# jlk9/MPAS-Ocean.jl

Hardware: AMD Instinct MI355X
Metric: cell-updates/sec per RK4 step (higher is better)
Workload: dtype f64

## Files before the change

include/moka_hip.h:

```cpp
#ifndef MOKA_HIP_H
#define MOKA_HIP_H
#include <stdint.h>

#ifdef __cplusplus
extern "C" {
#endif

typedef struct moka_ctx   moka_ctx;
typedef struct moka_plan  moka_plan;
typedef struct moka_mesh  moka_mesh;
typedef struct moka_state moka_state;

typedef enum {
    MOKA_OK = 0,
    MOKA_ERR_ARG = -1,
    MOKA_ERR_HIP = -2,
    MOKA_ERR_NO_DEVICE = -3,
    MOKA_ERR_ALLOC = -4,
    MOKA_ERR_UNSUPPORTED = -5,
    MOKA_ERR_COMM = -6
} moka_status;

typedef enum {
    MOKA_ORDER_DEFAULT = 0,
// ... 95 lines not shown
int  moka_mesh_info_get(const moka_mesh *mesh, moka_mesh_info *info);

int moka_gradient_on_edge(moka_mesh *mesh, const double *scalarCell, double *gradEdge);
int moka_divergence_on_cell(moka_mesh *mesh, const double *vecEdge, double *tempEdge, double *divCell);
int moka_curl_on_vertex(moka_mesh *mesh, const double *vecEdge, double *curlVertex);
int moka_interpolate_cell2edge(moka_mesh *mesh, const double *cellValue, double *edgeValue, int nlev);

int moka_gradient_on_edge_vjp(moka_mesh *mesh, double *dGradEdge , double *dScalarCell );
int moka_gradient_on_edge_jvp(moka_mesh *mesh, const double *dScalarCell, double *dGradEdge);
int moka_divergence_on_cell_vjp(moka_mesh *mesh, double *dDivCell , double *dVecEdge ,
                                double *dTempEdge );
int moka_divergence_on_cell_jvp(moka_mesh *mesh, const double *dVecEdge, double *dTempEdge , double *dDivCell);
int moka_curl_on_vertex_vjp(moka_mesh *mesh, const double *dCurlVertex, double *dVecEdge );
int moka_curl_on_vertex_jvp(moka_mesh *mesh, const double *dVecEdge, double *dCurlVertex );

int  moka_state_create(moka_ctx *ctx, moka_mesh *mesh, moka_state **out);
void moka_state_destroy(moka_state *st);
int  moka_state_upload(moka_state *st, int field, int time_level, const double *host);
int  moka_state_download(moka_state *st, int field, int time_level, double *host);

int  moka_state_download_rows(moka_state *st, int field, int time_level, int64_t nRows, const int32_t *rows, double *host);

int  moka_state_array_address(moka_state *st, int field, int time_level, uint64_t *address);

int  moka_state_optimize_placement(moka_state *st, int max_tries, double *ms_before, double *ms_after);
typedef struct { int32_t field; double ms_old, ms_new; int32_t kept; } moka_placement_trial;
int  moka_state_placement_log(const moka_state *st, int32_t capacity, moka_placement_trial *out, int32_t *n);
int64_t moka_state_placement_launches(const moka_state *st);

int moka_advance_time_levels(moka_state *st, int flags);
int moka_diagnostic_compute(moka_state *st, int flags);
int moka_compute_normal_velocity_tendency(moka_state *st, int flags);
int moka_compute_layer_thickness_tendency(moka_state *st, int flags);
int moka_tendencies(moka_state *st);
int moka_step_fe(moka_state *st, double dt, int flags);
int moka_step_rk4(moka_state *st, double dt);
int moka_run(moka_state *st, int integrator, double dt, int64_t nsteps, int flags);
int moka_sum_sq(moka_state *st, int field, int time_level, double *out);

typedef struct moka_halo moka_halo;
int  moka_ctx_streams(moka_ctx *ctx, void **compute_stream, void **comm_stream);
int  moka_mesh_permutation(const moka_mesh *mesh, int kind, int32_t *new_to_old);
int  moka_mesh_class_ranges(const moka_mesh *mesh, int32_t capacity, int32_t *nClasses, int32_t *patchStart,
                            int32_t *cellStart, int32_t *edgeStart);
int  moka_halo_create(moka_state *st, int32_t nNeighbors, const int32_t *sendCells, const int64_t *sendCellOff,
                      const int32_t *sendEdges, const int64_t *sendEdgeOff, const int32_t *recvCells,
// ... 158 lines not shown
```

mpas-ocean.jl_amd/csrc/api.hip:

```cpp
#include <hip/hip_runtime.h>

#include <algorithm>
#include <atomic>
#include <climits>
#include <cmath>
#include <cstdio>
#include <cstdlib>
#include <cstring>
#include <map>
#include <new>
#include <string>
#include <utility>
#include <vector>

#include "state.hpp"

namespace moka {

void fill_mesh_info(const Plan &p, moka_mesh_info *info);

struct TuningEntry {
    int mask, max;
    std::atomic<int> value;
    TuningEntry(int def, int m, int x) : mask(m), max(x), value(def) {}
    bool accepts(int v) const { return mask ? (v & ~mask) == 0 : v >= 0 && v <= max; }
};
static TuningEntry g_tuning[] = {
    {0, 0, -1},
    {1 << 0, 0x7f | 1 << 10 | 1 << 11, 0},
    {1, 0, 1},
    {1, 0, 1},
    {1, 0, 1},
    {0, 0, 3},
    {0, 0, INT_MAX},
    {0, 0, 1},
    {1 << 0 | 1 << 1 | 1 << 7, 0xf | 7 << 7 | 1 << 16, 0},
    {1, 0, 1},
};
constexpr int N_TUNING = sizeof(g_tuning) / sizeof(g_tuning[0]);

int tuning(TuningKey key) { return g_tuning[key].value.load(); }

}

namespace mk {

int fail(moka_ctx *ctx, int code, const std::string &msg)
{
    set_error(msg);
    if (ctx) ctx->err = msg;
    return code;
}

int lanes_per_column(int K)
{
    int l = 1;
    while (l < K && l < 64) l <<= 1;
    return l;
}

// ... 288 lines not shown
    const uint32_t rowB = 480;
    const int64_t nRows = bytes / rowB, nFetch = nRows / 4;
    uint32_t *sink = reinterpret_cast<uint32_t *>(static_cast<unsigned char *>(buf) + bytes);
    double best = 0.0;
    hipError_t rc = hipMemsetAsync(buf, 0x5A, (size_t)bytes + 64, s);
    for (int i = 0; i < iters && rc == hipSuccess; ++i) {
        if ((rc = hipEventRecord(ctx->ev0, s)) != hipSuccess) break;
        if ((rc = launch_bw_gather_n(buf, nRows, rowB, nFetch, sink, ctx->nCUs, s)) != hipSuccess) break;
        if ((rc = hipEventRecord(ctx->ev1, s)) != hipSuccess) break;
        if ((rc = hipEventSynchronize(ctx->ev1)) != hipSuccess) break;
        float ms = 0.f;
        if ((rc = hipEventElapsedTime(&ms, ctx->ev0, ctx->ev1)) != hipSuccess) break;
        best = std::max(best, (double)nFetch * rowB / ((double)ms * 1e-3) / 1e9);
    }
    (void)hipStreamSynchronize(s);
    (void)hipFree(buf);
    HIPCHK(ctx, rc);
    *gbs = best;
    return MOKA_OK;
}

int moka_set_tuning(int key, int value)
{
    if (key < 1 || key >= N_TUNING) return fail(nullptr, MOKA_ERR_ARG, "unknown tuning key");
    if (!g_tuning[key].accepts(value)) return fail(nullptr, MOKA_ERR_ARG, "tuning key " + std::to_string(key) + ": value names no kernel instance");
    g_tuning[key].value.store(value);
    return MOKA_OK;
}

int moka_get_tuning(int key, int *value)
{
    if (!value) return fail(nullptr, MOKA_ERR_ARG, "value is NULL");
    if (key < 1 || key >= N_TUNING) return fail(nullptr, MOKA_ERR_ARG, "unknown tuning key");
    *value = g_tuning[key].value.load();
    return MOKA_OK;
}

int moka_kernel_variant_available(int variant)
{
    return variant == 0 || variant == 3 || variant == 4 || variant == 11;
}

int moka_set_kernel_variant(moka_ctx *ctx, int variant)
{
    if (!ctx) return fail(nullptr, MOKA_ERR_ARG, "ctx is NULL");
    if (variant < 0 || variant > 14) return fail(ctx, MOKA_ERR_ARG, "variant must be 0..14");
    if (!moka_kernel_variant_available(variant))
        return fail(ctx, MOKA_ERR_UNSUPPORTED, "this kernel variant was an experiment of rounds 1-3 and no longer exists (0, 3, 4, 11 do)");
    ctx->variant = variant;
    return MOKA_OK;
}

int moka_mesh_create(moka_ctx *ctx, const moka_mesh_desc *desc, moka_mesh **out)
{
    if (!ctx || !out) return fail(ctx, MOKA_ERR_ARG, "NULL argument");
    *out = nullptr;
// ... 252 lines not shown
```

mpas-ocean.jl_amd/csrc/api_state.hip:

```cpp
#include <hip/hip_runtime.h>

#include <algorithm>
#include <cmath>
#include <climits>
#include <cstdint>
#include <mutex>
#include <new>
#include <string>
#include <unordered_set>
#include <utility>
#include <vector>

#include "state.hpp"
#include "tapes.hpp"

namespace mk {

static std::mutex g_liveMutex;
static std::unordered_set<const moka_state *> g_liveStates;
void state_attach(moka_state *st, bool halo)
{
    std::lock_guard<std::mutex> lk(g_liveMutex);
    if (g_liveStates.count(st)) { ++st->attached; st->halos += halo; }
}
bool state_detach(moka_state *st, bool halo)
{
    std::lock_guard<std::mutex> lk(g_liveMutex);
    const bool alive = g_liveStates.count(st) != 0;
    if (alive) { --st->attached; st->halos -= halo; }
    return alive;
}

int ensure_rk_bufs(moka_state *st)
{
    if (st->rk[1].ssh) return MOKA_OK;
    const Plan &p = st->mesh->plan;
    LevelBufs tmp[2];
    const size_t mark = st->mem.mark();
    const size_t sb = st->f32 ? 4 : 8;
    int rc = MOKA_OK;
    for (auto &r : tmp) {
        if (rc == MOKA_OK) rc = st->mem.alloc(&r.u, (size_t)p.K * p.nE, sb);
        if (rc == MOKA_OK) rc = st->mem.alloc(&r.h, (size_t)p.K * p.nC, sb);
        if (rc == MOKA_OK) rc = st->mem.alloc(&r.ssh, (size_t)p.nC, sb);
    }
    if (rc != MOKA_OK) {
        st->mem.rollback(mark);
        return rc;
    }
    st->rk[0] = tmp[0]; st->rk[1] = tmp[1];
    st->phys[2] = tmp[0]; st->phys[3] = tmp[1];
    return MOKA_OK;
}

int ensure_spare(moka_state *st)
{
    if (st->spare.ssh) return MOKA_OK;
    const Plan &p = st->mesh->plan;
    LevelBufs tmp;
    const size_t mark = st->mem.mark();
    const size_t sb = st->f32 ? 4 : 8;
    int rc = st->mem.alloc(&tmp.u, (size_t)p.K * p.nE, sb);
    if (rc == MOKA_OK) rc = st->mem.alloc(&tmp.h, (size_t)p.K * p.nC, sb);
    if (rc == MOKA_OK) rc = st->mem.alloc(&tmp.ssh, (size_t)p.nC, sb);
    if (rc != MOKA_OK) {
        st->mem.rollback(mark);
        return rc;
    }
    st->spare = tmp;
    st->phys[4] = tmp;
    return MOKA_OK;
}

LevelBufs &fe_new_level(moka_state *st) { return st->spare.ssh ? st->spare : st->lev[0]; }

void fe_rotate_levels(moka_state *st)
{
    if (st->spare.ssh) {
        const LevelBufs oldPrev = st->lev[0];
        st->lev[0] = st->lev[1];
// ... 427 lines not shown
int moka_state_create(moka_ctx *ctx, moka_mesh *mesh, moka_state **out)
{
    if (!ctx || !mesh || !out) return fail(ctx, MOKA_ERR_ARG, "NULL argument");
    *out = nullptr;
    moka_state *st = new (std::nothrow) moka_state();
    if (!st) return fail(ctx, MOKA_ERR_ALLOC, "out of host memory");
    st->ctx = ctx;
    st->mem.ctx = ctx;
    st->mesh = mesh;
    const Plan &p = mesh->plan;
    HIPCHK(ctx, hipSetDevice(ctx->device));
    const size_t nEK = (size_t)p.K * p.nE, nCK = (size_t)p.K * p.nC, nVK = (size_t)p.K * p.nV;
    st->f32 = p.stateBytes == 4;
    const MeshDev launchDev = launch_bounds(mesh);
    if (st->f32 && !stage_f32_supported(launchDev)) {
        delete st;
        return fail(ctx, MOKA_ERR_UNSUPPORTED,
                    "fp32-storage state: needs nVertLevels % 4 == 0, nVertLevels <= 128, fields below 4 GiB and patches whose "
                    "records + own u rows fit 64 KB of LDS (smaller patch_cells)");
    }
    const size_t sb = st->f32 ? 4 : 8;
    int rc = MOKA_OK;
    auto A = [&](double **q, size_t n, size_t eb = 8) { if (rc == MOKA_OK) rc = st->mem.alloc(q, n, eb); };
    for (auto &l : st->lev) { A(&l.ssh, p.nC, sb); A(&l.u, nEK, sb); A(&l.h, nCK, sb); }
    A(&st->hEdge[0], nEK, sb); A(&st->hEdge[1], nEK, sb);
    A(&st->F, nEK, sb); A(&st->div, nCK, sb); A(&st->vort, nVK, sb);
    A(&st->tendU, nEK, sb); A(&st->tendH, nCK, sb);
    A(&st->scalar, 2);
    if (rc != MOKA_OK) { moka_state_destroy(st); return rc; }
    st->phys[0] = st->lev[0]; st->phys[1] = st->lev[1];
    HIPCHK(ctx, hipStreamSynchronize(ctx->stream));
    {
        std::lock_guard<std::mutex> lk(g_liveMutex);
        g_liveStates.insert(st);
    }
    *out = st;
    return MOKA_OK;
}

void moka_state_destroy(moka_state *st)
{
    if (!st) return;
    {
        std::lock_guard<std::mutex> lk(g_liveMutex);
        g_liveStates.erase(st);
    }
    (void)hipSetDevice(st->ctx->device);
// ... 511 lines not shown
```

mpas-ocean.jl_amd/csrc/halo.hip:

```cpp
#include <fcntl.h>
#include <sys/mman.h>
#include <sys/stat.h>
#include <unistd.h>

#include <algorithm>
#include <chrono>
#include <cerrno>
#include <cstring>
#include <new>
#include <string>
#include <thread>
#include <vector>

#include "state.hpp"

using namespace mk;

namespace {

struct PushDst {
    unsigned char *u, *h, *ssh;
};

struct PeerLink {
// ... 242 lines not shown
                     const int64_t *recvCellOff, const int32_t *recvEdges, const int64_t *recvEdgeOff,
                     int32_t nPatchesBoundary, int32_t nPatchesOwned, moka_halo **out)
{
    if (!st || !out || nNeighbors < 0 || !sendCellOff || !sendEdgeOff || !recvCellOff || !recvEdgeOff)
        return fail(st ? st->ctx : nullptr, MOKA_ERR_ARG, "NULL argument");
    *out = nullptr;
    const Plan &p = st->mesh->plan;
    if (st->viscDel4 != 0.0)
        return fail(st->ctx, MOKA_ERR_UNSUPPORTED, "Del4 mixing: not on a state with a halo (its stencil reaches three cell rings, the nonlinear halo two)");
    if (st->nTracers > 0) return fail(st->ctx, MOKA_ERR_UNSUPPORTED, "tracers: whole meshes only (no halo; moka_set_tracers(st, 0) first)");
    if (mom_vmix_on(st)) return fail(st->ctx, MOKA_ERR_UNSUPPORTED, "vertical momentum mixing: whole meshes only (no halo; switch the pass off first)");
    if (st->forcedTapes > 0) return fail(st->ctx, MOKA_ERR_UNSUPPORTED, "a moka_forced_tape of this state exists: whole meshes only (no halo)");
    if (nNeighbors > 60) return fail(st->ctx, MOKA_ERR_ARG, "at most 60 neighbours");
    if (nPatchesBoundary < 0 || nPatchesOwned < nPatchesBoundary || nPatchesOwned > p.nPatches)
        return fail(st->ctx, MOKA_ERR_ARG, "patch ranges must satisfy 0 <= boundary <= owned <= nPatches");
    {
        const auto &cp = p.classPatchStart;
        const bool okB = std::find(cp.begin(), cp.end(), nPatchesBoundary) != cp.end();
        const bool okO = std::find(cp.begin(), cp.end(), nPatchesOwned) != cp.end();
        if (!okB || !okO)
            return fail(st->ctx, MOKA_ERR_ARG, "boundary / owned patch counts must be class boundaries of the mesh (moka_mesh_class_ranges)");
    }
    HIPCHK(st->ctx, hipSetDevice(st->ctx->device));
    if (int rc = ensure_rk_bufs(st)) return rc;
    if (int rc = ensure_spare(st)) return rc;
    moka_halo *h = new (std::nothrow) moka_halo();
    if (!h) return fail(st->ctx, MOKA_ERR_ALLOC, "out of host memory");
    h->st = st;
    h->mem.ctx = st->ctx;
    h->nNbr = nNeighbors;
    h->pBoundary = nPatchesBoundary; h->pOwned = nPatchesOwned;
    h->pFirst = nPatchesBoundary;
    h->overlapB = nPatchesBoundary > 0 && nPatchesOwned - nPatchesBoundary < 12000;
    int rc = MOKA_OK;
    try {
        if ((rc = build_halo_map(h, nNeighbors, sendCells, sendCellOff, sendEdges, sendEdgeOff, &h->sendMap, &h->nSend)) ||
            (rc = build_halo_map(h, nNeighbors, recvCells, recvCellOff, recvEdges, recvEdgeOff, &h->recvMap, &h->nRecv))) {
            moka_halo_destroy(h);
            return rc;
        }
        h->peers.resize(nNeighbors);
        h->recvCellStart.assign(nNeighbors, 0); h->recvCellCount.assign(nNeighbors, 0);
        h->recvEdgeStart.assign(nNeighbors, 0); h->recvEdgeCount.assign(nNeighbors, 0);
        h->sendCellCount.resize(nNeighbors); h->sendEdgeCount.resize(nNeighbors);
        for (int i = 0; i < nNeighbors; ++i) {
            h->sendCellCount[i] = (int32_t)(sendCellOff[i + 1] - sendCellOff[i]);
// ... 167 lines not shown
}

int moka_halo_set_acquire(moka_halo *h, int on)
{
    if (!h) return fail(nullptr, MOKA_ERR_ARG, "halo is NULL");
    h->acquireFence = on != 0;
    return MOKA_OK;
}

int moka_halo_direct_available(const moka_halo *h)
{
    return h && h->directOk ? 1 : 0;
}

int moka_halo_export(moka_halo *h, int32_t nbr, int32_t shared, moka_halo_peer_info *out)
{
    if (!h || !out) return fail(h ? h->st->ctx : nullptr, MOKA_ERR_ARG, "NULL argument");
    if (nbr < 0 || nbr >= h->nNbr) return hfail(h, MOKA_ERR_ARG, "neighbour index out of range");
    if (!h->directOk) return hfail(h, MOKA_ERR_UNSUPPORTED, "direct halo transport unavailable: " + h->directWhy);
    moka_state *st = h->st;
    HIPCHK(st->ctx, hipSetDevice(st->ctx->device));
    if (int rc = ensure_flags(h, shared != 0)) return rc;
    if (shared && h->shmName.empty()) return hfail(h, MOKA_ERR_ARG, "the flag block of this halo was created process-local");
    std::memset(out, 0, sizeof *out);
    for (int t = 0; t < moka_state::NPHYS; ++t) {
        void *ptrs[3] = {st->phys[t].u, st->phys[t].h, st->phys[t].ssh};
        for (int f = 0; f < 3; ++f) {
            out->ptr[3 * t + f] = (uint64_t)(uintptr_t)ptrs[f];
            if (shared) {
                hipIpcMemHandle_t hd;
                HIPCHK(st->ctx, hipIpcGetMemHandle(&hd, ptrs[f]));
                static_assert(sizeof hd <= sizeof out->ipc[0], "IPC handle larger than its slot");
                std::memcpy(out->ipc[3 * t + f], &hd, sizeof hd);
            }
        }
    }
    out->flagPtr = (uint64_t)(uintptr_t)h->flags;
    std::strncpy(out->shmName, h->shmName.c_str(), sizeof out->shmName - 1);
    out->dstCell = h->recvCellStart[nbr]; out->dstEdge = h->recvEdgeStart[nbr];
    out->nCells = h->recvCellCount[nbr]; out->nEdges = h->recvEdgeCount[nbr];
    out->slot = nbr;
    out->nNeighbors = h->nNbr;
    out->pid = (int32_t)getpid();
    out->device = st->ctx->device;
    out->stateBytes = st->f32 ? 4 : 8;
    out->nVertLevels = st->mesh->plan.K;
// ... 478 lines not shown
```

mpas-ocean.jl_amd/csrc/inspect.hip:

```cpp
#include <algorithm>

#include "state.hpp"

using namespace mk;

namespace {

template <class T>
__global__ __launch_bounds__(256) void k_gather_rows(double *dst, const T *src, const int32_t *rows, int64_t n, int K)
{
    const int64_t total = n * K;
    for (int64_t i = (int64_t)blockIdx.x * 256 + threadIdx.x; i < total; i += (int64_t)gridDim.x * 256) {
        const int64_t r = i / K;
        const int k = (int)(i - r * K);
        dst[i] = (double)src[(int64_t)rows[r] * K + k];
    }
}

}

extern "C" int moka_state_download_rows(moka_state *st, int field, int time_level, int64_t nRows, const int32_t *rows, double *host)
{
    if (!st || (nRows > 0 && (!rows || !host)) || nRows < 0) return fail(st ? st->ctx : nullptr, MOKA_ERR_ARG, "NULL argument or nRows < 0");
    moka_ctx *c = st->ctx;
// ... 54 lines not shown
    hipError_t e = hipMemcpyAsync(dRows, lib.data(), (size_t)nRows * sizeof(int32_t), hipMemcpyHostToDevice, s);
    if (e == hipSuccess) {
        const unsigned blocks = (unsigned)std::min<int64_t>((nRows * K + 255) / 256, 16384);
        if (st->f32) hipLaunchKernelGGL(k_gather_rows<float>, dim3(blocks), dim3(256), 0, s, dOut, reinterpret_cast<const float *>(src), dRows, nRows, K);
        else hipLaunchKernelGGL(k_gather_rows<double>, dim3(blocks), dim3(256), 0, s, dOut, src, dRows, nRows, K);
        e = hipGetLastError();
    }
    if (e == hipSuccess) e = hipMemcpyAsync(host, dOut, (size_t)nRows * K * sizeof(double), hipMemcpyDeviceToHost, s);
    if (e == hipSuccess) e = hipStreamSynchronize(s);
    if (e != hipSuccess) return done(fail(c, MOKA_ERR_HIP, std::string("moka_state_download_rows: ") + hipGetErrorString(e)));
    return done(MOKA_OK);
}

extern "C" int moka_state_array_address(moka_state *st, int field, int time_level, uint64_t *address)
{
    if (!st || !address) return fail(st ? st->ctx : nullptr, MOKA_ERR_ARG, "NULL argument");
    if (time_level < 0 || time_level > 3 || field < MOKA_F_SSH || field > MOKA_F_LAYER_THICKNESS)
        return fail(st->ctx, MOKA_ERR_ARG, "prognostic fields, time_level 0..3");
    const LevelBufs &b = time_level < 2 ? st->lev[time_level] : st->rk[time_level - 2];
    const double *q = field == MOKA_F_SSH ? b.ssh : field == MOKA_F_NORMAL_VELOCITY ? b.u : b.h;
    *address = (uint64_t)(uintptr_t)q;
    return MOKA_OK;
}
```

mpas-ocean.jl_amd/csrc/kernels.hpp:

```cpp
#pragma once
#include <hip/hip_runtime.h>

#include <initializer_list>

#include "moka_internal.hpp"

namespace moka {

struct StageArgs {
    const double *pu, *ph;
    const double *ssh;
    const double *cu, *ch;
    const double *nu_in, *nh_in;
    double *nu_out, *nh_out;
    double *pu_out, *ph_out;
    double *ssh_out;
    double *tendU, *tendH;
    double a, b;
    int feMode;
    const double *hEdgeOld;
    const double *hPrev;
    double *hEdgeNew, *F, *div;
    const double *areaCell;
    double *vort;
// ... 42 lines not shown
    const double *auxD = nullptr;
    int auxW = 0;
};

hipError_t launch_stage(const MeshDev &m, const StageArgs &a, int lpc, hipStream_t s);
hipError_t launch_stage_col(const MeshDev &m, const StageArgs &a, hipStream_t s);
hipError_t launch_stage_rec2c(const MeshDev &m, const StageArgs &a, hipStream_t s);
bool rec2c_supported(const MeshDev &m);
bool stage_curl_fused(const MeshDev &m);
bool stage_curl_fits(const MeshDev &m, bool f32);
bool stage_f32_supported(const MeshDev &m);
hipError_t launch_stage_rec2c_f32(const MeshDev &m, const StageArgs &a, hipStream_t s);

enum TuningKey : int {
    TUNE_F32_WIDE = 1,
    TUNE_FE_PREV = 2,
    TUNE_CURL_FUSED = 3,
    TUNE_FE_LEAN = 4,
    TUNE_NL_SHAPE = 5,
    TUNE_NL_CAP = 6,
    TUNE_RK13 = 7,
    TUNE_PAIR = 8,
    TUNE_FE_LEAN_INST = 9,
};
int tuning(TuningKey key);

hipError_t raise_dyn_lds(std::initializer_list<const void *> fns, int bytes);
hipError_t launch_update_ssh_f32(const MeshDev &m, const float *h, float *ssh, int nlev, int lpc, hipStream_t s);
hipError_t launch_permute_rows_f32(void *dst, const void *src, const int32_t *n2o, int64_t n, int K, int to_device,
                                   hipStream_t s);
hipError_t launch_halo_map_f32(float *buf, float *h, float *ssh, float *u, const uint32_t *map, int64_t n, int unpack,
                               hipStream_t s);
hipError_t launch_fe(const MeshDev &m, const FeArgs &a, int lpc, hipStream_t s);
hipError_t launch_curl2(const MeshDev &m, const double *u, double *vort, bool accum, hipStream_t s);
hipError_t launch_curl_f32(const MeshDev &m, const float *u, float *vort, bool accum, hipStream_t s);
hipError_t launch_operator(const MeshDev &m, const OpArgs &a, int lpc, hipStream_t s);
hipError_t launch_update_ssh(const MeshDev &m, const double *h, double *ssh, int nlev, int lpc, hipStream_t s);
hipError_t launch_permute_rows(double *dst, const double *src, const int32_t *n2o, int64_t n, int K, int to_device,
                               hipStream_t s);
hipError_t launch_sum_sq_serial(const double *a, int64_t n, double *out, hipStream_t s);
hipError_t launch_copy(double *dst, const double *src, int64_t n, hipStream_t s);
hipError_t launch_bw_copy(void *dst, const void *src, int64_t bytes, int nCUs, hipStream_t s);
hipError_t launch_bw_streams(void *buf, int64_t bytes, hipStream_t s);
hipError_t launch_bw_gather_n(const void *src, int64_t nRows, uint32_t rowB, int64_t nFetch, uint32_t *sink, int nCUs, hipStream_t s);
hipError_t launch_bw_read(const void *src, int64_t bytes, uint32_t *sink, int nCUs, hipStream_t s);
hipError_t launch_bw_gather(const void *src, int64_t bytes, uint32_t rowB, uint32_t *sink, int nCUs, hipStream_t s);
// ... 181 lines not shown
```

mpas-ocean.jl_amd/csrc/placement.hip:

```cpp
#include <algorithm>
#include <cmath>
#include <cstring>

#include "state.hpp"

using namespace mk;

namespace {

struct FieldSlot {
    int id;
    int set;
    int which;
    unsigned stages;
};
const FieldSlot kSlots[12] = {{6, 2, 0, 0xF}, {9, 3, 0, 0x6}, {3, 1, 0, 0xF}, {0, 0, 0, 0xF},
                              {7, 2, 1, 0xF}, {10, 3, 1, 0x6}, {4, 1, 1, 0xF}, {1, 0, 1, 0xF},
                              {8, 2, 2, 0xF}, {11, 3, 2, 0x6}, {5, 1, 2, 0x8}, {2, 0, 2, 0x1}};
constexpr int NSLOTS = 12;

LevelBufs &set_of(moka_state *st, int set) { return set == 0 ? st->lev[1] : set == 1 ? st->lev[0] : st->rk[set - 2]; }

void repoint(moka_state *st, double *oldp, double *newp)
{
    auto fix = [&](LevelBufs &b) {
        if (b.u == oldp) b.u = newp;
        if (b.h == oldp) b.h = newp;
        if (b.ssh == oldp) b.ssh = newp;
    };
    for (auto &b : st->lev) fix(b);
    for (auto &b : st->rk) fix(b);
    fix(st->spare);
    for (auto &b : st->phys) fix(b);
    for (void *&q : st->mem.ptrs) if (q == (void *)oldp) q = (void *)newp;
}

struct Timer {
    hipEvent_t ev[5] = {nullptr, nullptr, nullptr, nullptr, nullptr};
    ~Timer() { for (hipEvent_t e : ev) if (e) (void)hipEventDestroy(e); }
};

int time_stages(moka_state *st, Timer &T, int reps, double ms[4])
{
    moka_ctx *c = st->ctx;
    std::vector<float> v[4];
    for (int r = -1; r < reps; ++r) {
        for (int s = 1; s <= 4; ++s) {
            if (r >= 0) HIPCHK(c, hipEventRecord(T.ev[s - 1], c->stream));
            HIPCHK(c, run_stage(st, rk4_stage_args(st, s, 0.0, st->lev[1].ssh)));
            ++st->placementLaunches;
        }
        if (r < 0) continue;
        HIPCHK(c, hipEventRecord(T.ev[4], c->stream));
        HIPCHK(c, hipEventSynchronize(T.ev[4]));
        for (int s = 0; s < 4; ++s) {
            float t = 0.f;
            HIPCHK(c, hipEventElapsedTime(&t, T.ev[s], T.ev[s + 1]));
            v[s].push_back(t);
// ... 120 lines not shown
        if (keep) {
            double again[4];
            repoint(st, static_cast<double *>(cand), oldp);
            rc = time_stages(st, T, REPS, again);
            repoint(st, oldp, static_cast<double *>(cand));
            if (rc) {
                repoint(st, static_cast<double *>(cand), oldp);
                (void)hipStreamSynchronize(s);
                (void)hipFree(cand);
                (void)restore();
                cleanup();
                return rc;
            }
            for (int k = 0; k < 4; ++k) if (f.stages >> k & 1u) best[k] = std::min(best[k], again[k]);
            was = over(best, f.stages);
            keep = now < was * (1.0 - 0.004);
        }
        moka_placement_trial log{f.id, was, now, keep ? 1 : 0};
        st->placementLog.push_back(log);
        void *loser = keep ? (void *)oldp : cand;
        if (keep) {
            for (int k = 0; k < 4; ++k) if (f.stages >> k & 1u) best[k] = ms[k];
            sinceGain = 0;
        } else {
            repoint(st, static_cast<double *>(cand), oldp);
            ++sinceGain;
        }
        held.push_back({loser, bytes});
        heldBytes += bytes;
    }
    hipError_t er = restore();
    cleanup();
    if (er != hipSuccess) return fail(c, MOKA_ERR_HIP, std::string("restoring the previous time level: ") + hipGetErrorString(er));
    if (ms_after) *ms_after = over(best, 0xF);
    return MOKA_OK;
}

int64_t moka_state_placement_launches(const moka_state *st) { return st ? st->placementLaunches : 0; }

int moka_state_placement_log(const moka_state *st, int32_t capacity, moka_placement_trial *out, int32_t *n)
{
    if (!st || !n) return fail(st ? st->ctx : nullptr, MOKA_ERR_ARG, "NULL argument");
    *n = (int32_t)st->placementLog.size();
    for (int32_t i = 0; out && i < capacity && i < *n; ++i) out[i] = st->placementLog[i];
    return MOKA_OK;
}

}
```

mpas-ocean.jl_amd/csrc/state.hpp:

```cpp
#pragma once
#include <hip/hip_runtime.h>

#include <algorithm>
#include <initializer_list>
#include <map>
#include <string>
#include <utility>
#include <vector>

#include "kernels.hpp"
#include "moka_internal.hpp"

struct moka_ctx {
    int device = 0;
    hipStream_t stream = nullptr;
    hipStream_t comm = nullptr;
    hipEvent_t ev0 = nullptr, ev1 = nullptr;
    hipEvent_t evBoundary = nullptr, evInterior = nullptr, evHalo = nullptr;
    int variant = 0;
    int nCUs = 256;
    std::string err;
    bool stageTiming = false;
    std::vector<hipEvent_t> evPool;
    size_t evUsed = 0;
    std::vector<hipEvent_t> marks;
    size_t marksUsed = 0;
    void *bwBuf = nullptr;
    size_t bwBytes = 0;
};

namespace mk {

int fail(moka_ctx *ctx, int code, const std::string &msg);
int h2d(moka_ctx *ctx, void *dst, const void *src, size_t bytes);
// ... 132 lines not shown
    int halos = 0;
    int nTracers = 0;
    double *trPhi[2] = {nullptr, nullptr}, *trProv[2] = {nullptr, nullptr};
    int tracerPath = 0;
    std::vector<double> trKappa;
    double *trKappaDev = nullptr;
    std::vector<double> trKappa4;
    double *trKappa4Dev = nullptr, *trLap = nullptr;
    std::vector<double> trKappaV;
    double *trKappaVDev = nullptr, *trVmixScratch = nullptr;
    int vmixPath = 0;
    std::vector<double *> trVf;
    std::vector<char> trVfOn;
    std::vector<uint64_t> trVfGen;
    uint64_t trVfClock = 0;
    double **trVfDev = nullptr;
    std::vector<double *> trSrc;
    double **trSrcDev = nullptr;
    double momNuV = 0.0, momDrag = 0.0;
    double *momTau = nullptr, *momScratch = nullptr;
    bool momTauOn = false;
    int momVmixPath = 0;
    mk::DeviceAllocs mem;
    int attached = 0;
    int dycoreTapes = 0;
    int forcedTapes = 0;
    int64_t forcedSteps = 0;
    std::vector<moka_placement_trial> placementLog;
    int64_t placementLaunches = 0;
};

namespace mk {

using namespace moka;

void state_attach(moka_state *st, bool halo = false);
bool state_detach(moka_state *st, bool halo = false);

inline bool default_stage_kernels(const moka_state *st)
{
    const int v = st->ctx->variant;
    return (v == 0 || v == 11) && st->mesh->lpc == 64 && st->mesh->colOk;
}
inline MeshDev launch_bounds(const moka_mesh *mm)
{
    MeshDev dev = mm->dev;
    dev.maxOwnE = std::max(mm->plan.maxOwnELaunch, 1); dev.maxOwnC = std::max(mm->plan.maxOwnCLaunch, 1);
    return dev;
}
inline bool mom_vmix_on(const moka_state *st) { return st->momNuV != 0.0 || st->momDrag != 0.0 || (st->momTau && st->momTauOn); }
inline int nl_form(const moka_ctx *ctx) { return ctx->variant == 4 ? 1 : ctx->variant == 3 ? 3 : 0; }

int ensure_op_bufs(moka_mesh *m);
const int32_t *perm_of(const moka_mesh *m, int kind);
int put_rows(moka_mesh *m, double *dst, const double *host, int kind, int64_t n, int K, bool f32 = false);
int get_rows(moka_mesh *m, double *host, const double *src, int kind, int64_t n, int K, bool f32 = false);
int ensure_rk_bufs(moka_state *st);
int ensure_spare(moka_state *st);
LevelBufs &fe_new_level(moka_state *st);
void fe_rotate_levels(moka_state *st);
int flush_lazy(moka_state *st, bool diag, bool tend);
hipError_t run_stage(moka_state *st, const StageArgs &g, int pBegin = 0, int pCount = -1, hipStream_t on = nullptr, int tail = -1);
StageArgs rk4_stage_args(moka_state *st, int s, double dt, const double *ssh0);
LevelBufs &rk4_stage_output(moka_state *st, int s);
int rk4_begin(moka_state *st, const double **ssh0);
void rk4_end(moka_state *st);
bool rk13_usable(const moka_state *st);
StageArgs rk13_stage_args(moka_state *st, int s, double dt, const double *ssh0);
void rk13_end(moka_state *st);
FeArgs fe_args(moka_state *st, int ops, int flags, double dt);
StageArgs fe_stage_args(moka_state *st, const FeArgs &a, int flags);
bool fe_stage_path(const moka_state *st, int flags);
bool fe_lean(const moka_state *st, int flags);
int fe_begin(moka_state *st, int flags);
void fe_end(moka_state *st, int flags, bool stageKernel, bool lean, bool prevMode);
int step_rk4(moka_state *st, double dt, moka_tracer_tape *rec);
int momentum_vmix(moka_state *st, double *u, const double *h, double dt);
hipError_t tracer_stage(moka_state *st, int s, const StageArgs &g);
int tracer_vmix(moka_mesh *mm, moka_ctx *ctx, int nT, const double *h, double *x, const double *kv, const double *const *fld, double dt,
                double *scratch, bool reverse, int *path, const int32_t *gslot = nullptr, const double *p_new = nullptr, double *D = nullptr);
bool vfield_on(const moka_state *st, int j);
// ... 4 lines not shown
```

mpas-ocean.jl_amd/moka_hip/lib.py:

```python
from __future__ import annotations

import ctypes as C
import os
import subprocess

import numpy as np

PKG_DIR = os.path.dirname(os.path.dirname(os.path.abspath(__file__)))
LIB_PATH = os.environ.get("MOKA_HIP_LIB") or os.path.join(PKG_DIR, "libmoka_hip.so")

_i32p = C.POINTER(C.c_int32)
_f64p = C.POINTER(C.c_double)

OK = 0
ERR_ARG, ERR_HIP, ERR_NO_DEVICE, ERR_ALLOC, ERR_UNSUPPORTED, ERR_COMM = -1, -2, -3, -4, -5, -6
ORDER_DEFAULT, ORDER_NONE, ORDER_RCM, ORDER_RCB = 0, 1, 2, 3
TRACER_GRAD_KAPPA, TRACER_GRAD_KAPPA4 = 1, 2
VGRAD_INTERFACE, VGRAD_CELL, VGRAD_PROFILE = 0, 1, 2
FORCED_GRAD_STRESS, FORCED_GRAD_VISCOSITY, FORCED_GRAD_DRAG = 1, 2, 4
CELL, EDGE, VERTEX = 0, 1, 2
(F_SSH, F_NORMAL_VELOCITY, F_LAYER_THICKNESS, F_LAYER_THICKNESS_EDGE, F_THICKNESS_FLUX,
 F_VELOCITY_DIV_CELL, F_RELATIVE_VORTICITY, F_TEND_NORMAL_VELOCITY, F_TEND_LAYER_THICKNESS) = range(9)
FE_STALE_HEDGE, FE_ACCUM_VORT, FE_LEVEL1_ONLY, FE_REFERENCE_COMPAT = 1, 2, 4, 7
FORWARD_EULER, RUNGE_KUTTA_4 = 0, 1
# ... 52 lines not shown
    "moka_version", "moka_ctx_create", "moka_ctx_destroy", "moka_last_error", "moka_sync",
    "moka_timer_start", "moka_timer_stop",
    "moka_plan_create", "moka_plan_destroy", "moka_plan_info", "moka_plan_permutation", "moka_plan_patch_ranges", "moka_plan_array",
    "moka_mesh_create", "moka_mesh_destroy", "moka_mesh_info_get",
    "moka_gradient_on_edge", "moka_divergence_on_cell", "moka_curl_on_vertex", "moka_interpolate_cell2edge",
    "moka_state_create", "moka_state_destroy", "moka_state_upload", "moka_state_download",
    "moka_advance_time_levels", "moka_diagnostic_compute", "moka_compute_normal_velocity_tendency",
    "moka_compute_layer_thickness_tendency", "moka_tendencies", "moka_step_fe", "moka_step_rk4", "moka_run",
    "moka_sum_sq", "moka_set_kernel_variant", "moka_kernel_variant_available", "moka_stage_timing", "moka_stage_timing_read",
    "moka_ctx_streams", "moka_halo_create", "moka_halo_destroy", "moka_halo_buffer_elems", "moka_halo_pack",
    "moka_halo_unpack", "moka_rk4_dist_begin", "moka_rk4_dist_stage", "moka_rk4_dist_end",
    "moka_plan_class_ranges", "moka_mesh_class_ranges", "moka_mesh_permutation", "moka_halo_direct_available", "moka_halo_set_overlap", "moka_halo_pack_fields", "moka_halo_unpack_fields",
    "moka_tape_record_rk4", "moka_tape_commit_rk4", "moka_adjoint_rk4_stage_fields", "moka_adjoint_rk4_stage",
    "moka_tape_record_fe", "moka_tape_commit_fe", "moka_adjoint_fe_step_fields", "moka_adjoint_fe_step",
    "moka_halo_export", "moka_halo_connect", "moka_halo_push_begin", "moka_halo_push_signal", "moka_halo_push_wait",
    "moka_rk4_dist_stage_launch", "moka_rk4_dist_step", "moka_fe_dist_launch", "moka_fe_dist_end", "moka_fe_dist_step",
    "moka_set_nonlinear", "moka_last_fe_path", "moka_set_viscosity_del2", "moka_set_viscosity_del4", "moka_state_del4_path", "moka_tape_create", "moka_tape_destroy", "moka_step_fe_taped", "moka_step_rk4_taped", "moka_adjoint_seed_sum_sq_ssh", "moka_adjoint_sweep",
    "moka_adjoint_download",
    "moka_mark", "moka_marks_reset", "moka_marks_read", "moka_bw_probe", "moka_bw_probe_streams", "moka_bw_probe_reread", "moka_bw_probe_gather_big", "moka_ctx_pci_bus_id", "moka_halo_set_acquire", "moka_set_tuning", "moka_get_tuning", "moka_rk4_dist_parts_available", "moka_adjoint_rk4_stage_part", "moka_adjoint_rk4_parts_available", "moka_adjoint_rk4_stage_out_fields",
    "moka_gradient_on_edge_vjp", "moka_gradient_on_edge_jvp", "moka_divergence_on_cell_vjp", "moka_divergence_on_cell_jvp",
    "moka_curl_on_vertex_vjp", "moka_curl_on_vertex_jvp", "moka_fe_lazy_pending",
    "moka_state_optimize_placement", "moka_state_placement_log", "moka_state_download_rows",
    "moka_halo_stats_enable", "moka_halo_stats_read", "moka_halo_set_stream_flags", "moka_state_array_address", "moka_state_placement_launches",
    "moka_state_rk4_streams",
    "moka_set_tracers", "moka_tracer_upload", "moka_tracer_download", "moka_state_tracer_path",
    "moka_set_tracer_diffusion", "moka_tracer_diffusion",
    "moka_set_tracer_biharmonic", "moka_tracer_biharmonic",
    "moka_set_tracer_vertical_diffusion", "moka_tracer_vertical_diffusion", "moka_state_tracer_vmix_path", "moka_tracer_adjoint_vmix_path",
    "moka_tracer_source_upload", "moka_tracer_source_download", "moka_tracer_has_source",
    "moka_tracer_vertical_field_upload", "moka_tracer_vertical_field_download", "moka_tracer_has_vertical_field",
    "moka_set_vertical_viscosity", "moka_vertical_viscosity", "moka_surface_stress_upload", "moka_surface_stress_download",
    "moka_has_surface_stress", "moka_state_momentum_vmix_path",
    "moka_tracer_adjoint_want_source_gradient", "moka_tracer_adjoint_source_download",
    "moka_tracer_adjoint_want_diffusivity_gradient", "moka_tracer_adjoint_diffusivity_gradient",
    "moka_tracer_adjoint_diffusivity_density_download",
    "moka_tracer_adjoint_want_vertical_gradient", "moka_tracer_adjoint_vertical_gradient",
    "moka_tracer_adjoint_vertical_density_download",
    "moka_tracer_tape_create", "moka_tracer_tape_destroy", "moka_step_rk4_tracer_taped", "moka_tracer_tape_steps",
    "moka_tracer_adjoint_seed", "moka_tracer_adjoint_sweep", "moka_tracer_adjoint_download", "moka_tracer_adjoint_path",
    "moka_forced_tape_create", "moka_forced_tape_destroy", "moka_step_rk4_forced_taped", "moka_forced_adjoint_seed_sum_sq_ssh",
    "moka_forced_adjoint_seed", "moka_forced_adjoint_sweep", "moka_forced_adjoint_download", "moka_forced_adjoint_want_gradient",
    "moka_forced_adjoint_density_download", "moka_forced_adjoint_gradient", "moka_forced_tape_vmix_path",
]


def build(force: bool = False) -> str:
    if force:
# ... 37 lines not shown
    L.moka_mesh_create.argtypes = [vp, C.POINTER(MeshDesc), C.POINTER(vp)]
    L.moka_mesh_destroy.argtypes = [vp]
    L.moka_mesh_destroy.restype = None
    L.moka_mesh_info_get.argtypes = [vp, C.POINTER(MeshInfo)]
    L.moka_gradient_on_edge.argtypes = [vp, _f64p, _f64p]
    L.moka_divergence_on_cell.argtypes = [vp, _f64p, _f64p, _f64p]
    L.moka_curl_on_vertex.argtypes = [vp, _f64p, _f64p]
    L.moka_interpolate_cell2edge.argtypes = [vp, _f64p, _f64p, C.c_int]
    L.moka_gradient_on_edge_vjp.argtypes = [vp, _f64p, _f64p]
    L.moka_gradient_on_edge_jvp.argtypes = [vp, _f64p, _f64p]
    L.moka_divergence_on_cell_vjp.argtypes = [vp, _f64p, _f64p, _f64p]
    L.moka_divergence_on_cell_jvp.argtypes = [vp, _f64p, _f64p, _f64p]
    L.moka_curl_on_vertex_vjp.argtypes = [vp, _f64p, _f64p]
    L.moka_curl_on_vertex_jvp.argtypes = [vp, _f64p, _f64p]
    L.moka_state_create.argtypes = [vp, vp, C.POINTER(vp)]
    L.moka_state_destroy.argtypes = [vp]
    L.moka_state_destroy.restype = None
    L.moka_state_optimize_placement.argtypes = [vp, C.c_int, _f64p, _f64p]
    L.moka_state_placement_launches.argtypes = [vp]
    L.moka_state_rk4_streams.argtypes = [vp]
    L.moka_state_placement_launches.restype = C.c_int64
    L.moka_state_placement_log.argtypes = [vp, C.c_int32, C.POINTER(PlacementTrial), _i32p]
    L.moka_state_array_address.argtypes = [vp, C.c_int, C.c_int, C.POINTER(C.c_uint64)]
    L.moka_state_download_rows.argtypes = [vp, C.c_int, C.c_int, C.c_int64, _i32p, _f64p]
    L.moka_state_upload.argtypes = [vp, C.c_int, C.c_int, _f64p]
    L.moka_state_download.argtypes = [vp, C.c_int, C.c_int, _f64p]
    L.moka_advance_time_levels.argtypes = [vp, C.c_int]
    L.moka_diagnostic_compute.argtypes = [vp, C.c_int]
    L.moka_compute_normal_velocity_tendency.argtypes = [vp, C.c_int]
    L.moka_compute_layer_thickness_tendency.argtypes = [vp, C.c_int]
    L.moka_tendencies.argtypes = [vp]
    L.moka_step_fe.argtypes = [vp, C.c_double, C.c_int]
    L.moka_step_rk4.argtypes = [vp, C.c_double]
    L.moka_run.argtypes = [vp, C.c_int, C.c_double, C.c_int64, C.c_int]
    L.moka_sum_sq.argtypes = [vp, C.c_int, C.c_int, _f64p]
    L.moka_set_kernel_variant.argtypes = [vp, C.c_int]
    L.moka_kernel_variant_available.argtypes = [C.c_int]
    L.moka_stage_timing.argtypes = [vp, C.c_int]
    L.moka_stage_timing_read.argtypes = [vp, C.POINTER(C.c_double), C.POINTER(C.c_int64)]
    L.moka_ctx_streams.argtypes = [vp, C.POINTER(vp), C.POINTER(vp)]
    i64p = C.POINTER(C.c_int64)
    L.moka_halo_create.argtypes = [vp, C.c_int32, _i32p, i64p, _i32p, i64p, _i32p, i64p, _i32p, i64p,
                                   C.c_int32, C.c_int32, C.POINTER(vp)]
    L.moka_halo_destroy.argtypes = [vp]
    L.moka_halo_set_stream_flags.argtypes = [vp, C.c_int]
    L.moka_halo_stats_enable.argtypes = [vp, C.c_int]
# ... 254 lines not shown
```

Baseline: 9.176 billion.

## Place prognostic time-level arrays in a staggered contiguous device slab

```diff
diff --git a/include/moka_hip.h b/include/moka_hip.h
--- a/include/moka_hip.h
+++ b/include/moka_hip.h
@@ -141,6 +141,8 @@
 int  moka_state_download_rows(moka_state *st, int field, int time_level, int64_t nRows, const int32_t *rows, double *host);
 
 int  moka_state_array_address(moka_state *st, int field, int time_level, uint64_t *address);
+int  moka_state_slab_info(const moka_state *st, int region, uint64_t *base, uint64_t *bytes, uint64_t *plan_offset, uint64_t *granule);
+uint64_t moka_slab_array_offset(int set, int kind, int64_t nEdges, int64_t nCells, int nVertLevels, int elemBytes, int64_t granule);
 
 int  moka_state_optimize_placement(moka_state *st, int max_tries, double *ms_before, double *ms_after);
 typedef struct { int32_t field; double ms_old, ms_new; int32_t kept; } moka_placement_trial;
diff --git a/mpas-ocean.jl_amd/csrc/api.hip b/mpas-ocean.jl_amd/csrc/api.hip
--- a/mpas-ocean.jl_amd/csrc/api.hip
+++ b/mpas-ocean.jl_amd/csrc/api.hip
@@ -24,6 +24,7 @@
     std::atomic<int> value;
     TuningEntry(int def, int m, int x) : mask(m), max(x), value(def) {}
     bool accepts(int v) const { return mask ? (v & ~mask) == 0 : v >= 0 && v <= max; }
+    bool exists() const { return mask != 0 || max >= 0; }
 };
 static TuningEntry g_tuning[] = {
     {0, 0, -1},
@@ -36,6 +37,10 @@
     {0, 0, 1},
     {1 << 0 | 1 << 1 | 1 << 7, 0xf | 7 << 7 | 1 << 16, 0},
     {1, 0, 1},
+    {0, 0, -1},
+    {0, 0, -1},
+    {1, 0, 1},
+    {mk::SLAB_GRANULE_DEFAULT_UNITS, 0, mk::SLAB_GRANULE_MAX_UNITS},
 };
 constexpr int N_TUNING = sizeof(g_tuning) / sizeof(g_tuning[0]);
 
@@ -370,7 +375,7 @@
 
 int moka_set_tuning(int key, int value)
 {
-    if (key < 1 || key >= N_TUNING) return fail(nullptr, MOKA_ERR_ARG, "unknown tuning key");
+    if (key < 1 || key >= N_TUNING || !g_tuning[key].exists()) return fail(nullptr, MOKA_ERR_ARG, "unknown tuning key");
     if (!g_tuning[key].accepts(value)) return fail(nullptr, MOKA_ERR_ARG, "tuning key " + std::to_string(key) + ": value names no kernel instance");
     g_tuning[key].value.store(value);
     return MOKA_OK;
@@ -379,7 +384,7 @@
 int moka_get_tuning(int key, int *value)
 {
     if (!value) return fail(nullptr, MOKA_ERR_ARG, "value is NULL");
-    if (key < 1 || key >= N_TUNING) return fail(nullptr, MOKA_ERR_ARG, "unknown tuning key");
+    if (key < 1 || key >= N_TUNING || !g_tuning[key].exists()) return fail(nullptr, MOKA_ERR_ARG, "unknown tuning key");
     *value = g_tuning[key].value.load();
     return MOKA_OK;
 }
diff --git a/mpas-ocean.jl_amd/csrc/api_state.hip b/mpas-ocean.jl_amd/csrc/api_state.hip
--- a/mpas-ocean.jl_amd/csrc/api_state.hip
+++ b/mpas-ocean.jl_amd/csrc/api_state.hip
@@ -31,9 +31,86 @@
     return alive;
 }
 
+SlabPlan slab_plan_of(const moka_state *st)
+{
+    const Plan &p = st->mesh->plan;
+    return slab_plan((size_t)p.nE, (size_t)p.nC, (size_t)p.K, st->f32 ? 4 : 8, st->slabGranule);
+}
+
+bool in_slab(const moka_state *st, const void *q)
+{
+    if (!st->slabOn) return false;
+    const SlabPlan sp = slab_plan_of(st);
+    for (int r = 0; r < SLAB_REGIONS; ++r) {
+        const char *b = static_cast<const char *>(st->slab[r]);
+        if (b && static_cast<const char *>(q) >= b && static_cast<const char *>(q) < b + sp.regionBytes[r]) return true;
+    }
+    return false;
+}
+
+static int slab_region(moka_state *st, int region)
+{
+    const SlabPlan sp = slab_plan_of(st);
+    void *base = nullptr;
+    if (int rc = st->mem.take(&base, sp.regionBytes[region], true)) return rc;
+    st->slab[region] = base;
+    for (int set = 0; set < SLAB_SETS; ++set) {
+        if (slab_region_of(set) != region) continue;
+        auto at = [&](int kind) { return reinterpret_cast<double *>(static_cast<char *>(base) + (sp.offset[set][kind] - sp.regionBegin[region])); };
+        st->phys[set].u = at(0); st->phys[set].h = at(1); st->phys[set].ssh = at(2);
+    }
+    return MOKA_OK;
+}
+
+void repoint(moka_state *st, double *oldp, double *newp)
+{
+    auto fix = [&](LevelBufs &b) {
+        if (b.u == oldp) b.u = newp;
+        if (b.h == oldp) b.h = newp;
+        if (b.ssh == oldp) b.ssh = newp;
+    };
+    for (auto &b : st->lev) fix(b);
+    for (auto &b : st->rk) fix(b);
+    fix(st->spare);
+    for (auto &b : st->phys) fix(b);
+    if (in_slab(st, oldp) || in_slab(st, newp)) return;
+    for (void *&q : st->mem.ptrs) if (q == (void *)oldp) q = (void *)newp;
+}
+
+int slab_release(moka_state *st)
+{
+    if (!st->slabOn) return MOKA_OK;
+    const SlabPlan sp = slab_plan_of(st);
+    const size_t mark = st->mem.mark();
+    std::vector<std::pair<double *, double *>> moved;
+    int rc = MOKA_OK;
+    for (int set = 0; set < SLAB_SETS && rc == MOKA_OK; ++set) {
+        double *arr[SLAB_KINDS] = {st->phys[set].u, st->phys[set].h, st->phys[set].ssh};
+        for (int kind = 0; kind < SLAB_KINDS && rc == MOKA_OK; ++kind) {
+            if (!arr[kind] || !in_slab(st, arr[kind])) continue;
+            void *fresh = nullptr;
+            if ((rc = st->mem.take(&fresh, sp.bytes[set][kind], false))) break;
+            const hipError_t e = hipMemcpyAsync(fresh, arr[kind], sp.bytes[set][kind], hipMemcpyDeviceToDevice, st->ctx->stream);
+            if (e != hipSuccess) rc = fail(st->ctx, MOKA_ERR_HIP, std::string("hipMemcpyAsync: ") + hipGetErrorString(e));
+            moved.push_back({arr[kind], static_cast<double *>(fresh)});
+        }
+    }
+    if (rc != MOKA_OK) { st->mem.rollback(mark); return rc; }
+    HIPCHK(st->ctx, hipStreamSynchronize(st->ctx->stream));
+    for (auto &m : moved) repoint(st, m.first, m.second);
+    for (void *&b : st->slab) st->mem.release(b);
+    st->slabOn = false;
+    return MOKA_OK;
+}
+
 int ensure_rk_bufs(moka_state *st)
 {
     if (st->rk[1].ssh) return MOKA_OK;
+    if (st->slabOn) {
+        if (int rc = slab_region(st, 1)) return rc;
+        st->rk[0] = st->phys[2]; st->rk[1] = st->phys[3];
+        return MOKA_OK;
+    }
     const Plan &p = st->mesh->plan;
     LevelBufs tmp[2];
     const size_t mark = st->mem.mark();
@@ -56,6 +133,11 @@
 int ensure_spare(moka_state *st)
 {
     if (st->spare.ssh) return MOKA_OK;
+    if (st->slabOn) {
+        if (int rc = slab_region(st, 2)) return rc;
+        st->spare = st->phys[4];
+        return MOKA_OK;
+    }
     const Plan &p = st->mesh->plan;
     LevelBufs tmp;
     const size_t mark = st->mem.mark();
@@ -529,7 +611,14 @@
     const size_t sb = st->f32 ? 4 : 8;
     int rc = MOKA_OK;
     auto A = [&](double **q, size_t n, size_t eb = 8) { if (rc == MOKA_OK) rc = st->mem.alloc(q, n, eb); };
-    for (auto &l : st->lev) { A(&l.ssh, p.nC, sb); A(&l.u, nEK, sb); A(&l.h, nCK, sb); }
+    st->slabOn = tuning(TUNE_SLAB) != 0;
+    st->slabGranule = (size_t)tuning(TUNE_SLAB_GRANULE) * SLAB_GRANULE_UNIT;
+    if (st->slabOn) {
+        rc = slab_region(st, 0);
+        st->lev[0] = st->phys[0]; st->lev[1] = st->phys[1];
+    } else {
+        for (auto &l : st->lev) { A(&l.ssh, p.nC, sb); A(&l.u, nEK, sb); A(&l.h, nCK, sb); }
+    }
     A(&st->hEdge[0], nEK, sb); A(&st->hEdge[1], nEK, sb);
     A(&st->F, nEK, sb); A(&st->div, nCK, sb); A(&st->vort, nVK, sb);
     A(&st->tendU, nEK, sb); A(&st->tendH, nCK, sb);
diff --git a/mpas-ocean.jl_amd/csrc/halo.hip b/mpas-ocean.jl_amd/csrc/halo.hip
--- a/mpas-ocean.jl_amd/csrc/halo.hip
+++ b/mpas-ocean.jl_amd/csrc/halo.hip
@@ -288,6 +288,8 @@
             return fail(st->ctx, MOKA_ERR_ARG, "boundary / owned patch counts must be class boundaries of the mesh (moka_mesh_class_ranges)");
     }
     HIPCHK(st->ctx, hipSetDevice(st->ctx->device));
+    if (st->slabOn && st->attached == 0)
+        if (int rc = slab_release(st)) return rc;
     if (int rc = ensure_rk_bufs(st)) return rc;
     if (int rc = ensure_spare(st)) return rc;
     moka_halo *h = new (std::nothrow) moka_halo();
@@ -501,6 +503,8 @@
     HIPCHK(st->ctx, hipSetDevice(st->ctx->device));
     if (int rc = ensure_flags(h, shared != 0)) return rc;
     if (shared && h->shmName.empty()) return hfail(h, MOKA_ERR_ARG, "the flag block of this halo was created process-local");
+    if (shared && st->slabOn)
+        return hfail(h, MOKA_ERR_UNSUPPORTED, "the state's arrays sit in its slab (a tape existed when the halo was created): create the halo before the tape");
     std::memset(out, 0, sizeof *out);
     for (int t = 0; t < moka_state::NPHYS; ++t) {
         void *ptrs[3] = {st->phys[t].u, st->phys[t].h, st->phys[t].ssh};
diff --git a/mpas-ocean.jl_amd/csrc/inspect.hip b/mpas-ocean.jl_amd/csrc/inspect.hip
--- a/mpas-ocean.jl_amd/csrc/inspect.hip
+++ b/mpas-ocean.jl_amd/csrc/inspect.hip
@@ -100,3 +100,22 @@
     *address = (uint64_t)(uintptr_t)q;
     return MOKA_OK;
 }
+
+extern "C" int moka_state_slab_info(const moka_state *st, int region, uint64_t *base, uint64_t *bytes, uint64_t *plan_offset, uint64_t *granule)
+{
+    if (!st || region < 0 || region >= SLAB_REGIONS) return fail(st ? st->ctx : nullptr, MOKA_ERR_ARG, "NULL state or region outside 0..2");
+    if (!st->slabOn) return fail(st->ctx, MOKA_ERR_UNSUPPORTED, "this state's arrays are allocations of their own (no slab)");
+    const SlabPlan sp = slab_plan_of(st);
+    if (base) *base = (uint64_t)(uintptr_t)st->slab[region];
+    if (bytes) *bytes = sp.regionBytes[region];
+    if (plan_offset) *plan_offset = sp.regionBegin[region];
+    if (granule) *granule = st->slabGranule;
+    return MOKA_OK;
+}
+
+extern "C" uint64_t moka_slab_array_offset(int set, int kind, int64_t nEdges, int64_t nCells, int nVertLevels, int elemBytes, int64_t granule)
+{
+    if (set < 0 || set >= SLAB_SETS || kind < 0 || kind >= SLAB_KINDS || nEdges < 0 || nCells < 0 || nVertLevels < 1 || (elemBytes != 4 && elemBytes != 8) || granule < 0)
+        return UINT64_MAX;
+    return array_offset(set, kind, (size_t)nEdges, (size_t)nCells, (size_t)nVertLevels, (size_t)elemBytes, (size_t)granule);
+}
diff --git a/mpas-ocean.jl_amd/csrc/kernels.hpp b/mpas-ocean.jl_amd/csrc/kernels.hpp
--- a/mpas-ocean.jl_amd/csrc/kernels.hpp
+++ b/mpas-ocean.jl_amd/csrc/kernels.hpp
@@ -88,6 +88,8 @@
     TUNE_RK13 = 7,
     TUNE_PAIR = 8,
     TUNE_FE_LEAN_INST = 9,
+    TUNE_SLAB = 12,
+    TUNE_SLAB_GRANULE = 13,
 };
 int tuning(TuningKey key);
 
diff --git a/mpas-ocean.jl_amd/csrc/placement.hip b/mpas-ocean.jl_amd/csrc/placement.hip
--- a/mpas-ocean.jl_amd/csrc/placement.hip
+++ b/mpas-ocean.jl_amd/csrc/placement.hip
@@ -20,20 +20,6 @@
 constexpr int NSLOTS = 12;
 
 LevelBufs &set_of(moka_state *st, int set) { return set == 0 ? st->lev[1] : set == 1 ? st->lev[0] : st->rk[set - 2]; }
-
-void repoint(moka_state *st, double *oldp, double *newp)
-{
-    auto fix = [&](LevelBufs &b) {
-        if (b.u == oldp) b.u = newp;
-        if (b.h == oldp) b.h = newp;
-        if (b.ssh == oldp) b.ssh = newp;
-    };
-    for (auto &b : st->lev) fix(b);
-    for (auto &b : st->rk) fix(b);
-    fix(st->spare);
-    for (auto &b : st->phys) fix(b);
-    for (void *&q : st->mem.ptrs) if (q == (void *)oldp) q = (void *)newp;
-}
 
 struct Timer {
     hipEvent_t ev[5] = {nullptr, nullptr, nullptr, nullptr, nullptr};
@@ -200,12 +186,15 @@
         if (keep) {
             for (int k = 0; k < 4; ++k) if (f.stages >> k & 1u) best[k] = ms[k];
             sinceGain = 0;
+            if (in_slab(st, oldp)) { st->mem.ptrs.push_back(cand); loser = nullptr; }
         } else {
             repoint(st, static_cast<double *>(cand), oldp);
             ++sinceGain;
         }
-        held.push_back({loser, bytes});
-        heldBytes += bytes;
+        if (loser) {
+            held.push_back({loser, bytes});
+            heldBytes += bytes;
+        }
     }
     hipError_t er = restore();
     cleanup();
diff --git a/mpas-ocean.jl_amd/csrc/slab_plan.hpp b/mpas-ocean.jl_amd/csrc/slab_plan.hpp
--- /dev/null
+++ b/mpas-ocean.jl_amd/csrc/slab_plan.hpp
@@ -0,0 +1,56 @@
+#pragma once
+#include <cstddef>
+#include <cstdint>
+
+namespace mk {
+
+constexpr int SLAB_SETS = 5, SLAB_KINDS = 3, SLAB_REGIONS = 3;
+constexpr size_t SLAB_ALIGN = (size_t)2 << 20;
+constexpr size_t SLAB_GRANULE_UNIT = 256;
+constexpr int SLAB_GRANULE_MAX_UNITS = 512;
+constexpr int SLAB_GRANULE_DEFAULT_UNITS = 0;
+constexpr size_t SLAB_MODULI[] = {(size_t)4 << 10, (size_t)64 << 10, (size_t)2 << 20, (size_t)1 << 30};
+
+inline constexpr size_t slab_round_up(size_t x, size_t a) { return (x + a - 1) / a * a; }
+inline constexpr int slab_region_of(int set) { return set < 2 ? 0 : set < 4 ? 1 : 2; }
+inline constexpr int slab_stagger_index(int set, int kind) { return kind * SLAB_SETS + set; }
+inline constexpr size_t slab_array_bytes(int kind, size_t nE, size_t nC, size_t K, size_t elemBytes)
+{
+    const size_t b = kind == 0 ? nE * K * elemBytes : kind == 1 ? nC * K * elemBytes : nC * elemBytes;
+    return b < 16 ? 16 : b;
+}
+
+struct SlabPlan {
+    size_t offset[SLAB_SETS][SLAB_KINDS];
+    size_t bytes[SLAB_SETS][SLAB_KINDS];
+    size_t regionBegin[SLAB_REGIONS];
+    size_t regionBytes[SLAB_REGIONS];
+};
+
+inline SlabPlan slab_plan(size_t nE, size_t nC, size_t K, size_t elemBytes, size_t granule)
+{
+    SlabPlan p{};
+    size_t cursor = 0;
+    int region = -1;
+    for (int set = 0; set < SLAB_SETS; ++set)
+        for (int kind = 0; kind < SLAB_KINDS; ++kind) {
+            const size_t base = slab_round_up(cursor, SLAB_ALIGN);
+            if (slab_region_of(set) != region) {
+                if (region >= 0) p.regionBytes[region] = cursor - p.regionBegin[region];
+                region = slab_region_of(set);
+                p.regionBegin[region] = base;
+            }
+            p.offset[set][kind] = base + (size_t)slab_stagger_index(set, kind) * granule;
+            p.bytes[set][kind] = slab_array_bytes(kind, nE, nC, K, elemBytes);
+            cursor = p.offset[set][kind] + p.bytes[set][kind];
+        }
+    p.regionBytes[region] = cursor - p.regionBegin[region];
+    return p;
+}
+
+inline size_t array_offset(int role, int kind, size_t nE, size_t nC, size_t K, size_t elemBytes, size_t granule)
+{
+    return slab_plan(nE, nC, K, elemBytes, granule).offset[role][kind];
+}
+
+}
diff --git a/mpas-ocean.jl_amd/csrc/state.hpp b/mpas-ocean.jl_amd/csrc/state.hpp
--- a/mpas-ocean.jl_amd/csrc/state.hpp
+++ b/mpas-ocean.jl_amd/csrc/state.hpp
@@ -10,6 +10,7 @@
 
 #include "kernels.hpp"
 #include "moka_internal.hpp"
+#include "slab_plan.hpp"
 
 struct moka_ctx {
     int device = 0;
@@ -188,6 +189,9 @@
     bool momTauOn = false;
     int momVmixPath = 0;
     mk::DeviceAllocs mem;
+    bool slabOn = false;
+    size_t slabGranule = 0;
+    void *slab[mk::SLAB_REGIONS] = {nullptr, nullptr, nullptr};
     int attached = 0;
     int dycoreTapes = 0;
     int forcedTapes = 0;
@@ -223,6 +227,10 @@
 int get_rows(moka_mesh *m, double *host, const double *src, int kind, int64_t n, int K, bool f32 = false);
 int ensure_rk_bufs(moka_state *st);
 int ensure_spare(moka_state *st);
+SlabPlan slab_plan_of(const moka_state *st);
+bool in_slab(const moka_state *st, const void *p);
+void repoint(moka_state *st, double *oldp, double *newp);
+int slab_release(moka_state *st);
 LevelBufs &fe_new_level(moka_state *st);
 void fe_rotate_levels(moka_state *st);
 int flush_lazy(moka_state *st, bool diag, bool tend);
diff --git a/mpas-ocean.jl_amd/moka_hip/lib.py b/mpas-ocean.jl_amd/moka_hip/lib.py
--- a/mpas-ocean.jl_amd/moka_hip/lib.py
+++ b/mpas-ocean.jl_amd/moka_hip/lib.py
@@ -98,7 +98,7 @@
     "moka_curl_on_vertex_vjp", "moka_curl_on_vertex_jvp", "moka_fe_lazy_pending",
     "moka_state_optimize_placement", "moka_state_placement_log", "moka_state_download_rows",
     "moka_halo_stats_enable", "moka_halo_stats_read", "moka_halo_set_stream_flags", "moka_state_array_address", "moka_state_placement_launches",
-    "moka_state_rk4_streams",
+    "moka_state_rk4_streams", "moka_state_slab_info", "moka_slab_array_offset",
     "moka_set_tracers", "moka_tracer_upload", "moka_tracer_download", "moka_state_tracer_path",
     "moka_set_tracer_diffusion", "moka_tracer_diffusion",
     "moka_set_tracer_biharmonic", "moka_tracer_biharmonic",
@@ -182,6 +182,9 @@
     L.moka_state_placement_launches.restype = C.c_int64
     L.moka_state_placement_log.argtypes = [vp, C.c_int32, C.POINTER(PlacementTrial), _i32p]
     L.moka_state_array_address.argtypes = [vp, C.c_int, C.c_int, C.POINTER(C.c_uint64)]
+    L.moka_state_slab_info.argtypes = [vp, C.c_int] + [C.POINTER(C.c_uint64)] * 4
+    L.moka_slab_array_offset.argtypes = [C.c_int, C.c_int, C.c_int64, C.c_int64, C.c_int, C.c_int, C.c_int64]
+    L.moka_slab_array_offset.restype = C.c_uint64
     L.moka_state_download_rows.argtypes = [vp, C.c_int, C.c_int, C.c_int64, _i32p, _f64p]
     L.moka_state_upload.argtypes = [vp, C.c_int, C.c_int, _f64p]
     L.moka_state_download.argtypes = [vp, C.c_int, C.c_int, _f64p]
```

After: 9.175 billion (median of 2 runs). About the same (-0.0%).
